# SahakyanLab/GenomeAssembler_dev

Measured on AMD Instinct MI355X. Metric: k-mers built+scored/sec, higher is better.
Workload: dtype u64 keys / u32 counts / f64 scores; 1 GPU; cfg2 (configs[2]): 100 x 50000 bp segments per GPU, 150 bp reads at 50x, k=31, build + breakage scoring of all contigs; mode=segments, segments_total=100, distinct_kmers_rank0=3843627, parallelism=segments sharded over 1 GPU(s), no collective

## Files before the change

### genomeassembler_dev_amd/csrc/capi.hip

```cpp
#include <algorithm>
#include <atomic>
#include <functional>
#include <memory>
#include <mutex>
#include <new>
#include <thread>

#include "pipeline.h"
#include "scaffolds.h"

struct gasm_strlist {
    std::vector<char> data;
    std::vector<u64> off;
};

struct gasm_contigs {
    std::vector<char> data;
    std::vector<u64> off;
    u64 rows = 0;
    std::vector<u32> perm;
    int words = 1;
    std::vector<u64> dkeys;
    std::vector<u32> dmult;
};
// ... 731 lines not shown
    HIPCHK(hipStreamSynchronize(b->ctx->stream));
    *seg_read_off = b->h_sim_seg_off.data();
    *starts = b->h_read_start.data();
    return GASM_OK;
    API_GUARD_END
}

void gasm_batch_free(gasm_batch* b) {
    if (!b) return;
    b->d_read_start.release();
    (void)hipSetDevice(b->ctx->device);
    (void)hipStreamSynchronize(b->ctx->stream);
    for (StepSlot& x : b->slot) { if (x.cx && x.cx != b->ctx) (void)hipStreamSynchronize(x.cx->stream); x.bs.release(); x.dp.release(); x.ss.release(); }
    b->rd.release(); b->rd2.release(); b->guided.release(); b->d_rkc.release(); b->d_correct.release();
    for (ScoreTable& t : b->tb) t.release();
    for (ScoreTable& t : b->mtb) t.release();
    delete b;
}

static int batch_build(gasm_batch* b, const BuildOpts& o) {
    if (!b) { gasm_set_error("batch is null"); return GASM_ERR_INVALID; }
    GCHK(build_opts_check(o));
    b->built = false; b->scored = false;
    const bool pingpong = env_int("GASM_PINGPONG", 1) != 0;
    if (pingpong && b->slot[0].cx == nullptr && b->slot[1].cx == nullptr)
        b->n_slots = std::max(2, std::min(4, env_int("GASM_STEP_SLOTS", 3)));
    if (pingpong) {
        if (b->last_k && b->last_k != o.k) for (StepSlot& x : b->slot) if (x.cx) HIPCHK(hipStreamSynchronize(x.cx->stream));
        b->cur = (b->cur + 1) % b->n_slots;
    }
    StepSlot& st = b->S();
    st.paths_ready = false; st.ss.valid = false; st.ss.launched = false;
    if (o.strands == 2 && b->rd2.strands_of != b->rd.upload_id) GCHK(b->rd2.make_both_strands(st.cx, b->rd));
    GCHK(pipeline_build(st.cx, o.strands == 2 ? b->rd2 : b->rd, st.bs, o));
    b->last_k = o.k;
    b->built = true;
    return GASM_OK;
}

int gasm_batch_build(gasm_batch* b, int k, uint64_t genome_len_hint) {
    API_GUARD_BEGIN
    BuildOpts o;
    o.k = k; o.genome_len_hint = genome_len_hint;
    return batch_build(b, o);
    API_GUARD_END
}

int gasm_batch_build_solid(gasm_batch* b, int k, uint64_t genome_len_hint, uint32_t min_count) {
    API_GUARD_BEGIN
    BuildOpts o;
    o.k = k; o.genome_len_hint = genome_len_hint; o.min_count = min_count;
    return batch_build(b, o);
    API_GUARD_END
}

int gasm_batch_build_strands(gasm_batch* b, int k, uint64_t genome_len_hint, uint32_t min_count, uint32_t strands) {
    API_GUARD_BEGIN
    BuildOpts o;
    o.k = k; o.genome_len_hint = genome_len_hint; o.min_count = min_count; o.strands = strands;
    return batch_build(b, o);
    API_GUARD_END
}

int gasm_batch_build_tips(gasm_batch* b, int k, uint64_t genome_len_hint, uint32_t min_count, uint32_t strands, uint32_t tip_len, uint32_t tip_rounds) {
    API_GUARD_BEGIN
    BuildOpts o;
// ... 616 lines not shown
```

### genomeassembler_dev_amd/csrc/kernels.h

```cpp
#pragma once
#include <hip/hip_runtime.h>
#include <stdint.h>

#include "device_utils.h"
#include "keyops.h"

struct ReadSet {
    const u64* words;
    const u64* read_off;
    const u64* seg_read_off;
    const u32* seg_tile_start;
    const uint4* tile_info;
    u32 fixed_len;
    u32 n_segments;
};

__device__ __forceinline__ void read_span(const ReadSet& rs, u64 r, u64* p0, u32* len) {
    if (rs.fixed_len) { *p0 = rs.read_off ? rs.read_off[r] : r * rs.fixed_len; *len = rs.fixed_len; }
    else { const u64 a = rs.read_off[r]; *p0 = a; *len = (u32)(rs.read_off[r + 1] - a); }
}

struct GraphView {
    const void* dk_key;
    const u32* dstart;
// ... 121 lines not shown
__global__ void k_bucket_partition(ReadSet rs, const uint4* tinfo, int k, int bbits, u32 g, u32 padm, u32 n_tiles, const u64* bstart, u32* cursor,
                                   K* keys, u64 scratch, u32* flags);
template <class K, int TBL>
__global__ void k_bucket_dedup(K* keys, u32* mult, const u64* bstart, const u32* blen, u32* bucket_d, u32* overflow, u16* fdir, int low_bits, u32* dstart);
#define GASM_BUCKET_MAX 65535
template <class K>
__global__ void k_bucket_dedup_multi(const K* keys, K* keys_out, u32* mult, const u64* bstart, u32* bucket_d, u32* overflow, u16* fdir, int low_bits);
template <class K>
__global__ void k_bucket_solid(K* keys, u32* mult, const u64* bstart, u32* bucket_d, u16* fdir, int low_bits, int fbits, int bbits, u32 min_count,
                               u32* removed, u32* done, u32* dstart);
template <class K>
__global__ void k_tip_mark(GraphView gv, u32 n_segments, u32 chunks, const u8* eflag, const u32* clen, const u32* nxt, const u32* dk_cnt, const u64* bstart,
                           u32* mult, u32 tip_len, u32* flags, u32* tips);
template <class K>
__global__ void k_bubble_mark(GraphView gv, u32 n_segments, u32 chunks, const u8* eflag, const u32* clen, const u32* nxt, const u32* dk_cnt, const u64* bstart,
                              u32* mult, u32 bubble_len, u32* flags, u32* bubbles);
__global__ void k_kmer_spectrum(const u32* dstart, u32 nb, const u32* dk_cnt, u32 n_segments, u32 chunks, u32* hist);
template <class K>
__global__ void k_lowcov_mark(GraphView gv, u32 n_segments, u32 chunks, const u8* eflag, const u32* clen, const u32* nxt, const u32* dk_cnt, const u64* bstart,
                              u32* mult, u32 cov_len, u32 cov_cutoff, u32* flags, u32* removed);
__global__ void k_contig_cov(const u32* dstart, u32 nb, u32 n_segments, u32 chunks, const u64* link, const u32* e_cid, const u32* dk_cnt,
                             const u32* seg_cstart, unsigned long long* msum, u32* nedges);
template <class K>
__global__ void k_bucket_gather(const K* keys, const u32* mult, const u64* bstart, const u32* dstart, K* dk_key, u32* dk_cnt, u32* claim, u8* eflag,
                                u32* flags);
template <class K> __global__ void k_edge_target(GraphView gv, u32 n_segments, u32 chunks, u32* tgt, u32* claim);
__global__ void k_edge_multi(GraphView gv, u32 n_segments, u32 chunks, const u32* tgt, const u32* claim, u8* eflag);
template <class K>
__global__ void k_node_flags(GraphView gv, u32 n_segments, u32 chunks, const u32* claim, u8* eflag, u64* link, u32* clen);
__global__ void k_edge_next(GraphView gv, u32 n_segments, u32 chunks, const u32* tgt, const u8* eflag, u32* nxt, u64* link);
__global__ void k_link_jump(GraphView gv, u32 n_segments, u32 chunks, u64* link, const u32* prev_active, u32* active, int jumps, const u32* nxt,
                            u32* clen);
__global__ void k_rank_rulers(GraphView gv, u32 n_segments, u32 chunks, u64* link, u32* rtab, u32 rshift, u32* flags);
__global__ void k_rank_lds(GraphView gv, const u32* rtab, u64* link, int max_rounds, u32 rshift, u32 lds_entries, u32* flags);
__global__ void k_chain_len(const u32* nxt, const u64* link, u32* clen, const u32* n_edges_p);
__global__ void k_contig_scan(GraphView gv, const u8* eflag, const u32* clen, u32* e_cid, u64* e_coff, u32* seg_ncontig,
                              u64* seg_cbases, u32* done, u32* seg_cstart, u64* seg_bstart, const u32* flags, u32* report, u32 ticket);
__global__ void k_contig_place(GraphView gv, const u8* eflag, const u32* seg_cstart, const u64* seg_bstart, u32* e_cid, u64* e_coff,
                               u64* c_off, u32 n_segments, u32 chunks);
template <class K>
__global__ void k_contig_emit(GraphView gv, const u64* link, const u32* nxt, const u64* e_coff, u8* out, u32 n_segments, u32 chunks);
__global__ void k_reads_both_strands(const u64* words, const u64* read_off, const u64* seg_read_off, u32 fixed_len, u32 n_segments, u64 n_reads, u32 g,
                                     unsigned long long* out);
template <class K>
__global__ void k_contig_twin(GraphView gv, const u64* link, const u32* e_cid, const u64* c_off, const u32* seg_cstart, const u8* text, u32 n_segments,
                              u32* twin, u32* bad);

template <class K>
__global__ void k_pack_runs(const K* keys, const u32* mult, const u64* bstart, const u32* bucket_d, const u32* gb_list, const u64* dst_off, K* out_keys,
                            u32* out_cnt);
template <class K, int TBL>
__global__ void k_bucket_merge(const K* in_keys, const u32* in_cnt, const u64* run_off, const u32* run_len, u32 n_src, K* out_keys, u32* out_cnt,
                               const u64* bstart, u32* bucket_d, u32* overflow, u16* fdir, int low_bits, const u64* src_base);
__global__ void k_repack_reads(const u64* src, const u64* dir, u64* words_out);
__global__ void k_piece_positions(const u64* piece_first, const u64* piece_word_off, u32 n_pieces, u64 n_reads, u32 fixed_len, u64* pos);
__global__ void k_slice_last(const u32* a, const u64* off, u32 n, u32* out);

__global__ void k_chain_expand(const u64* cwords, const u64* c_off, const u64* sig_off, const u32* elem_contig, const u32* elem_skip, const u64* elem_pos,
                               const u64* out_off, u32 n_scaffolds, u64* out, u64 n_words);
struct ChainSigs {
    const u64* sig_off;
    const u32* elem_contig;
    const u32* elem_skip;
    const u64* elem_pos;
};
__global__ void k_str_bitonic(const u64* words, const u64* off, u32* idx, u32 n_pow2, u32 kk, u32 j, ChainSigs cs);
__global__ void k_str_bitonic_block(const u64* words, const u64* off, u32* idx, u32 n_pow2, u32 kk, u32 j0, ChainSigs cs);
__global__ void k_str_adjacent_eq(const u64* words, const u64* off, const u32* idx, u32 n, u8* same_as_prev, ChainSigs cs);
// ... 116 lines not shown
```

### genomeassembler_dev_amd/csrc/kernels_build.hip

```cpp
#include "device_utils.h"
#include "keyops.h"
#include "kernels.h"
#include "dedup_order.h"

typedef unsigned long long u64x2 __attribute__((ext_vector_type(2)));

typedef unsigned int u32x4nt __attribute__((ext_vector_type(4)));
__device__ __forceinline__ uint4 stream_load16(const uint4* p) {
    const u32x4nt v = __builtin_nontemporal_load(reinterpret_cast<const u32x4nt*>(p));
    return make_uint4(v.x, v.y, v.z, v.w);
}
__device__ __forceinline__ void stream_store16(u64x2 v, u64x2* p) { __builtin_nontemporal_store(v, p); }

__global__ void __launch_bounds__(GASM_WG) k_pack_ascii(const u8* __restrict__ ascii, u64 nbases_host, const u64* __restrict__ nbases_dev,
                                                        u64* __restrict__ words, u32* __restrict__ err) {
    const u64 nbases = nbases_dev ? *nbases_dev : nbases_host;
    const u64 nwords = (nbases + 31) / 32 + 4;
    bool ok = true;
    for (u64 t = (u64)blockIdx.x * GASM_WG + threadIdx.x; t < nwords; t += (u64)gridDim.x * GASM_WG) {
        const u64 b0 = t << 5;
        u64 w = 0;
        if (b0 + 32 <= nbases) {
            const uint4* src = reinterpret_cast<const uint4*>(ascii + b0);
            const uint4 v0 = src[0], v1 = src[1];
// ... 1010 lines not shown
    }
}

#define GASM_RANK_NONE 0xFFFFFFFFu
__global__ void __launch_bounds__(GASM_WG) k_rank_rulers(GraphView gv, u32 n_segments, u32 chunks, u64* __restrict__ link,
                                                         u32* __restrict__ rtab, u32 rshift, u32* __restrict__ flags) {
    const u32 rmask = (1u << rshift) - 1u;
    u32 seg, chunk;
    if (!seg_chunk(n_segments, chunks, &seg, &chunk)) return;
    const u32 nb = 1u << gv.bbits;
    const u32 lo = gv.dstart[seg * nb], hi = gv.dstart[(seg + 1) * nb];
    const u32 nr = (hi - lo + rmask) >> rshift;
    for (u32 r = chunk * GASM_WG + threadIdx.x; r < nr; r += chunks * GASM_WG) {
        const u32 i = lo + (r << rshift);
        u32 cur = i, acc = 0, e = GASM_RANK_NONE;
        int step = 0;
        for (; step < 4096; ++step) {
            const u64 l = link[cur];
            if (cur != i) link[cur] = ((u64)i << 32) | GASM_LINK_TAG | acc;
            const u32 a = (u32)(l >> 32);
            if (a == GASM_NONE32) break;
            acc += (u32)l & 0x7FFFFFFFu;
            const u32 al = a - lo;
            if ((l & GASM_LINK_DONE) || !(al & rmask)) { e = (al << 16) | acc; break; }
            if (a == i) break;
            cur = a;
        }
        if (step == 4096) flags[GASM_FLAG_RANK_FAILED] = 1u;
        rtab[(lo >> rshift) + seg + r] = e;
    }
}

#define GASM_RANK_DEAD 0x8000FFFFu
__global__ void __launch_bounds__(1024) k_rank_lds(GraphView gv, const u32* __restrict__ rtab, u64* __restrict__ link, int max_rounds,
                                                    u32 rshift, u32 lds_entries, u32* __restrict__ flags) {
    const u32 rmask = (1u << rshift) - 1u;
    extern __shared__ u32 s_e[];
    __shared__ u32 s_active;
    const u32 seg = blockIdx.x;
    const u32 nb = 1u << gv.bbits;
    const u32 lo = gv.dstart[seg * nb], hi = gv.dstart[(seg + 1) * nb];
    const u32 nr = (hi - lo + rmask) >> rshift;
    if (nr > lds_entries || hi - lo > 65534u) { if (threadIdx.x == 0) flags[GASM_FLAG_RANK_FAILED] = 1u; return; }
    const u32* src = rtab + (lo >> rshift) + seg;
    u32 mine[32];
    u32 live = 0;
#pragma unroll
    for (u32 q = 0; q < 32; ++q) {
        const u32 r = threadIdx.x + 1024 * q;
        u32 e = r < nr ? src[r] : GASM_RANK_NONE;
        bool hopping = false;
        if (e == GASM_RANK_NONE) e = GASM_RANK_DEAD;
        else {
            const u32 a = e >> 16;
            if ((a & rmask) || (a == (r << rshift) && !(e & 0xFFFFu))) e = (0x8000u | r) << 16;
            else if (a == (r << rshift)) e = GASM_RANK_DEAD;
            else { e = ((a >> rshift) << 16) | (e & 0xFFFFu); hopping = true; }
        }
        mine[q] = e;
        if (r < nr) s_e[r] = e;
        live |= (u32)hopping << q;
    }
    for (int round = 0; round < max_rounds; ++round) {
        if (threadIdx.x == 0) s_active = 0;
        __syncthreads();
        u32 any = 0;
// ... 22 lines not shown
        const bool go = s_active != 0;
        __syncthreads();
        if (!go) break;
    }
#pragma unroll
    for (u32 q = 0; q < 32; ++q) {
        const u32 r = threadIdx.x + 1024 * q;
        if (r >= nr) continue;
        const u32 e = mine[q];
        u64 l = ~0ull;
        if (!((live >> q) & 1u) && e != GASM_RANK_DEAD) {
            const u32 t = (e >> 16) & 0x7FFFu;
            if (s_e[t] != GASM_RANK_DEAD) {
                const u32 ot = src[t];
                l = ((u64)(lo + (ot >> 16)) << 32) | GASM_LINK_DONE | (((e & 0xFFFFu) + (ot & 0xFFFFu)) & 0xFFFFu);
            }
        }
        link[lo + (r << rshift)] = l;
    }
}

__global__ void __launch_bounds__(GASM_WG) k_chain_len(const u32* __restrict__ nxt, const u64* __restrict__ link, u32* __restrict__ clen,
                                                       const u32* __restrict__ n_edges_p) {
    const u32 n_edges = *n_edges_p;
    for (u32 i = blockIdx.x * GASM_WG + threadIdx.x; i < n_edges; i += gridDim.x * GASM_WG) {
        if (nxt[i] != GASM_NONE32) continue;
        const u64 l = link[i];
        const u32 a = (u32)(l >> 32);
        if (a == GASM_NONE32 || !(l & GASM_LINK_DONE)) continue;
        clen[a] = ((u32)l & 0x7FFFFFFFu) + 1;
    }
}

__global__ void __launch_bounds__(1024) k_contig_scan(GraphView gv, const u8* __restrict__ eflag, const u32* __restrict__ clen,
                                                      u32* __restrict__ e_cid, u64* __restrict__ e_coff,
                                                      u32* __restrict__ seg_ncontig, u64* __restrict__ seg_cbases,
                                                      u32* __restrict__ done, u32* __restrict__ seg_cstart, u64* __restrict__ seg_bstart,
                                                      const u32* __restrict__ flags, u32* __restrict__ report, u32 ticket) {
    __shared__ u32 s_last;
    __shared__ u32 s_cnt[16];
    __shared__ u64 s_bas[16];
    const u32 seg = blockIdx.x;
    const u32 nb = 1u << gv.bbits;
    const u32 lo = gv.dstart[seg * nb], hi = gv.dstart[(seg + 1) * nb];
    const u32 wv = threadIdx.x >> 6, ln = threadIdx.x & 63;
    const u32 per = ((hi - lo + 15) / 16 + 63) & ~63u;
    const u32 wa = min(hi, lo + wv * per), wb = min(hi, wa + per);
    u32 ccarry = 0;
    u64 bcarry = 0;
    for (u32 base = wa; base < wb; base += 1024) {
        u32 ef[16];
        u32 cl[16];
#pragma unroll
        for (u32 q = 0; q < 16; ++q) {
            const u32 i = base + q * 64 + ln;
            ef[q] = i < wb ? (u32)eflag[i] : 0u;
            cl[q] = i < wb ? clen[i] : 0u;
        }
#pragma unroll
        for (u32 q = 0; q < 16; ++q) __asm__ volatile("" : "+v"(cl[q]), "+v"(ef[q]));
#pragma unroll
        for (u32 q = 0; q < 16; ++q) {
            const u32 i = base + q * 64 + ln;
            const bool head = ef[q] & 1;
            const u32 len = head ? (u32)(gv.k - 1) + cl[q] : 0u;
            const u32 cinc = wave_incl_scan(head ? 1u : 0u);
            const u32 binc = wave_incl_scan(len);
            if (head) { e_cid[i] = ccarry + cinc - 1; e_coff[i] = bcarry + binc - len; }
            ccarry += wave_last(cinc);
            bcarry += wave_last(binc);
        }
    }
    if (ln == 0) { s_cnt[wv] = ccarry; s_bas[wv] = bcarry; }
    __syncthreads();
    u32 cbefore = 0, ctot = 0;
    u64 bbefore = 0, btot = 0;
#pragma unroll
    for (u32 w = 0; w < 16; ++w) {
        if (w < wv) { cbefore += s_cnt[w]; bbefore += s_bas[w]; }
        ctot += s_cnt[w]; btot += s_bas[w];
    }
    if (wv) {
        for (u32 base = wa + ln; base < wb; base += 2048) {
            u32 ef[32];
#pragma unroll
            for (u32 q = 0; q < 32; ++q) ef[q] = base + 64 * q < wb ? (u32)eflag[base + 64 * q] : 0u;
#pragma unroll
            for (u32 q = 0; q < 32; ++q)
                if (ef[q] & 1) { e_cid[base + 64 * q] += cbefore; e_coff[base + 64 * q] += bbefore; }
        }
    }
    if (threadIdx.x == 0) {
        publish_u32(&seg_ncontig[seg], ctot); publish_u64(&seg_cbases[seg], btot);
        s_last = count_in_last(done) ? 1u : 0u;
    }
    __syncthreads();
    if (!s_last || wv) return;
    seg_offsets_wave(seg_ncontig, seg_cbases, gridDim.x, seg_cstart, seg_bstart, gv.dstart, nb, flags, report, ticket);
}

__global__ void __launch_bounds__(GASM_WG) k_contig_place(GraphView gv, const u8* __restrict__ eflag,
                                                          const u32* __restrict__ seg_cstart, const u64* __restrict__ seg_bstart,
                                                          u32* __restrict__ e_cid, u64* __restrict__ e_coff,
                                                          u64* __restrict__ c_off, u32 n_segments, u32 chunks) {
    if (blockIdx.x == 0 && threadIdx.x == 0) c_off[seg_cstart[n_segments]] = seg_bstart[n_segments];
    for_seg_edges(gv.dstart, 1u << gv.bbits, n_segments, chunks, [&](u32 seg, u32, u32, u32 i) {
        if (!(eflag[i] & 1)) return;
        const u32 cid = seg_cstart[seg] + e_cid[i];
        const u64 off = seg_bstart[seg] + e_coff[i];
        e_cid[i] = cid;
        e_coff[i] = off;
        c_off[cid] = off;
    });
}

__device__ __forceinline__ u32 klow16(u64 a) { return (u32)a & 0xFFFFu; }
__device__ __forceinline__ u32 klow16(const K128& a) { return (u32)a.lo & 0xFFFFu; }
template <class K>
__global__ void __launch_bounds__(GASM_WG) k_contig_emit(GraphView gv, const u64* __restrict__ link, const u32* __restrict__ nxt,
                                                         const u64* __restrict__ e_coff, u8* __restrict__ out, u32 n_segments,
                                                         u32 chunks) {
    for_seg_edge_groups(gv.dstart, 1u << gv.bbits, n_segments, chunks, [&](u32, u32, u32, const u32 (&i)[GASM_EDGE_ILP], const bool (&ok)[GASM_EDGE_ILP]) {
        u64 l[GASM_EDGE_ILP], off[GASM_EDGE_ILP];
        u32 nx[GASM_EDGE_ILP];
        K key[GASM_EDGE_ILP];
        bool on[GASM_EDGE_ILP];
        const int k = gv.k;
        const bool wide = k >= 8;
#pragma unroll
        for (int q = 0; q < GASM_EDGE_ILP; ++q) {
            l[q] = ok[q] ? link[i[q]] : ~0ull;
            nx[q] = ok[q] ? nxt[i[q]] : 0u;
// ... 288 lines not shown
```

### genomeassembler_dev_amd/csrc/pipeline.h

```cpp
#pragma once
#include "gasm_internal.h"
#include "kernels.h"

template <class K> struct KeyTag { using type = K; };
template <class F> static inline int with_key(int words, F&& f) { return words == 1 ? f(KeyTag<u64>{}) : f(KeyTag<K128>{}); }
#define GLAUNCH_K(ctx, words, name, kern, grid, block, shmem, ...)          \
    GCHK(with_key(words, [&](auto _tag) -> int {                            \
        using K = typename decltype(_tag)::type;                            \
        GLAUNCH(ctx, name, kern, grid, block, shmem, __VA_ARGS__);          \
        return GASM_OK;                                                     \
    }))

struct DevReads {
    u32 n_segments = 0;
    u64 n_reads = 0, total_bases = 0;
    u32 fixed_len = 0;
    u32 min_len = 0, max_len = 0;
    u64 n_empty = 0;
    std::vector<u64> h_read_off;
    std::vector<u64> h_seg_read_off;
    std::vector<u64> h_seg_empty;
    bool positioned = false;
    int sim_shift = 52;
    u64 upload_id = 0;
// ... 75 lines not shown
    }
    template <class T> T* at(const DBuf& d, size_t i) const { return reinterpret_cast<T*>(static_cast<char*>(d.p) + t[i].off); }
};
struct PassState {
    DBuf d;
    std::vector<std::vector<u64>> h;
    bool queued = false;
    u32 param[2] = {0, 0};
    template <class T> const T* host(size_t i) const { return reinterpret_cast<const T*>(h[i].data()); }
};
enum { LINKS_SUCC, LINKS_PRED, LINKS_LSUP, LINKS_SSUP, LINKS_SKIPPED };
enum { PAIRS_REC, PAIRS_HIST, PAIRS_CNT };
enum { MAP_REC, MAP_PILE, MAP_HIST, MAP_CNT };
enum { MAPG_REC, MAPG_GAP, MAPG_PILE, MAPG_GPILE, MAPG_HIST, MAPG_CNT, MAPG_END, MAPG_ENDCNT };
enum { MAPSC_F64, MAPSC_I32, MAPSC_CNT, MAPSC_FX, MAPSC_PILE, MAPSC_COUNTERS };

struct BuildState {
    int k = 0, bbits = 0, fbits = 9, words = 1, bb_cap = 0;
    bool small_tbl = true;
    bool rank_global = false;
    bool single_pass = true;
    struct PartLayout {
        u64 reads_id = 0;
        int k = 0, bbits = 0, slack = 0, forced = 0;
        u32 padm = 0, g = 0;
        bool operator==(const PartLayout& o) const {
            return reads_id == o.reads_id && k == o.k && bbits == o.bbits && slack == o.slack && forced == o.forced && padm == o.padm && g == o.g;
        }
    } part;
    bool part_valid = false;
    u64 part_alloc = 0;
    bool multi_pass = false;
    bool ranked_in_lds = false;
    u32 tile_g = 1;
    u64 n_kmers = 0, hint = 0, reads_id = 0;
    BuildOpts opts;
    std::vector<u64> h_seg_nk;
    u64 D_cap = 0, maxD_cap = 0, bases_cap = 0;
    u32 maxD_est = 1, paths_est = 0;
    bool have_actual = false;
    u32 tile_orr = 1;
    bool part_single = false;
    bool scan_in_dedup = false;
    u32 ruler_shift = 0;
    u32 attempts_distinct = 0;
    u32 attempts_graph = 0;
    u32* h_report = nullptr;
    size_t h_report_words = 0;
    u32 ticket = 0;
    bool pending = false;
    u32 d_total = 0, n_contigs = 0;
    u64 contig_bases = 0;
    std::vector<u32> h_dstart;
    std::vector<u32> h_seg_cstart;
    std::vector<u64> h_seg_bstart;
    DBuf d_keys2;
    DBuf d_keys, d_mult, d_hist, d_toff, d_tcnt, d_fdir, d_bstart, d_bucket_d, d_dstart, d_flags, d_rtab;
    DBuf d_solid_removed;
    RoundStats round_stats[ROUND_KINDS] = {{GASM_MAX_TIP_ROUNDS}, {GASM_MAX_BUBBLE_ROUNDS}, {GASM_MAX_COV_ROUNDS}};
    DBuf d_ccov;
    std::vector<u64> h_ccov_m;
    std::vector<u32> h_ccov_n;
    bool coverage_queued = false;
    PassState links, pairs, map, mapg;
    PassState mapscore;
    int mapscore_shift[GASM_MAX_TABLES] = {};
// ... 100 lines not shown
```

### genomeassembler_dev_amd/csrc/pipeline.hip

```cpp
#include <atomic>
#include <chrono>
#include <thread>
#include "pipeline.h"

#include <algorithm>
#include <cmath>

__global__ void k_set_u64(u64* p, u64 v) { *p = v; }

__global__ void k_add_empty_reads(PathSet ps, const u64* __restrict__ seg_empty, u32* __restrict__ poscnt, u32* __restrict__ total) {
    const u32 seg = blockIdx.y;
    const u32 p = ps.seg_path_off[seg] + blockIdx.x * GASM_WG + threadIdx.x;
    if (p >= ps.seg_path_off[seg + 1]) return;
    const u32 e = (u32)seg_empty[seg];
    if (!e) return;
    if (ps.p_off[p + 1] > ps.p_off[p]) poscnt[ps.p_off[p]] += e;
    else total[p] += e;
}

struct Knobs {
    int dedup_tbl = 0, scatter_wgs = 8, hist_wgs = 64, rank_rounds = 18, bbits_add = 0, ruler_shift = 0;
    bool rank_global = false, sync_build = false;
    Knobs() {
        if (const char* v = getenv("GASM_DEDUP_TBL")) dedup_tbl = atoi(v);
        if (const char* v = getenv("GASM_SCATTER_WGS")) scatter_wgs = std::max(1, atoi(v));
        if (const char* v = getenv("GASM_HIST_WGS")) hist_wgs = std::max(1, atoi(v));
        if (const char* v = getenv("GASM_DBG_BBITS_ADD")) bbits_add = std::max(0, atoi(v));
        if (const char* v = getenv("GASM_RULER_SHIFT")) ruler_shift = std::min(4, std::max(0, atoi(v)));
        if (const char* v = getenv("GASM_DBG_RANK_ROUNDS")) rank_rounds = atoi(v);
        rank_global = getenv("GASM_RANK_GLOBAL") != nullptr;
        sync_build = getenv("GASM_SYNC_BUILD") != nullptr;
    }
};
static const Knobs& knobs() { static const Knobs k; return k; }

template <class T>
static int wait_word(gasm_ctx* ctx, const volatile T* word, T ticket) {
    const auto t0 = std::chrono::steady_clock::now();
    for (u32 spin = 0;; ++spin) {
        if (*word == ticket) { std::atomic_thread_fence(std::memory_order_acquire); return GASM_OK; }
        if ((spin & 1023u) == 1023u && std::chrono::steady_clock::now() - t0 > std::chrono::milliseconds(2)) break;
    }
    static const double limit_s = [] { const char* v = getenv("GASM_WAIT_TIMEOUT_S"); const double x = v && *v ? atof(v) : 300.0; return x > 0 ? x : 300.0; }();
    for (;;) {
        if (*word == ticket) { std::atomic_thread_fence(std::memory_order_acquire); return GASM_OK; }
        const hipError_t q = hipStreamQuery(ctx->stream);
        if (q == hipSuccess) break;
        if (q != hipErrorNotReady) { gasm_set_error("the stream failed while a report was awaited: %s", hipGetErrorString(q)); return GASM_ERR_HIP; }
        if (std::chrono::duration<double>(std::chrono::steady_clock::now() - t0).count() > limit_s) {
            gasm_set_error("no report from the device within %.0f s (GASM_WAIT_TIMEOUT_S): a kernel hangs or the GPU is lost", limit_s);
            return GASM_ERR_HIP;
        }
        std::this_thread::sleep_for(std::chrono::microseconds(50));
    }
    if (*word != ticket) { gasm_set_error("a kernel finished without writing its report"); return GASM_ERR_HIP; }
    std::atomic_thread_fence(std::memory_order_acquire);
    return GASM_OK;
}
int gasm_wait_word32(gasm_ctx* ctx, const volatile u32* word, u32 ticket) { return wait_word<u32>(ctx, word, ticket); }
int gasm_wait_word64(gasm_ctx* ctx, const volatile u64* word, u64 ticket) { return wait_word<u64>(ctx, word, ticket); }
static int wait_report(gasm_ctx* ctx, const volatile u32* word, u32 ticket) { return wait_word<u32>(ctx, word, ticket); }
// ... 338 lines not shown
    v.p_off = b_p_off ? b_p_off : d_p_off.as<u64>();
    v.seg_path_off = b_seg_path_off ? b_seg_path_off : d_seg_path_off.as<u32>();
    v.n_segments = n_segments;
    return v;
}

void DevPaths::release() { d_words.release(); d_p_off.release(); d_seg_path_off.release(); d_seg_base_off.release(); }

void BuildState::release() {
    for (DBuf* b : {&d_solid_removed, &d_ccov, &links.d, &pairs.d, &map.d, &mapg.d, &mapscore.d, &d_spectrum, &d_twin, &d_keys, &d_keys2, &d_mult, &d_hist, &d_toff, &d_tcnt, &d_fdir, &d_bstart, &d_bucket_d, &d_dstart, &d_flags, &d_dk_key, &d_dk_cnt,
                    &d_eflag, &d_nxt, &d_link, &d_clen, &d_ecid, &d_ecoff, &d_rtab, &d_seg_cbases, &d_seg_cstart,
                    &d_seg_bstart, &d_c_off, &d_contig_ascii})
        b->release();
    for (RoundStats& rs : round_stats) rs.d_stats.release();
    part_valid = false;
    if (h_report) { (void)hipHostFree(h_report); h_report = nullptr; h_report_words = 0; }
}

void ScoreState::release() {
    for (DBuf* b : {&d_tbl_off, &d_seed, &d_gpos, &d_poscnt, &d_total, &d_out_f64, &d_out_i32, &d_freq, &d_pd_off, &d_pd, &d_seg_empty, &d_fxsum, &d_first, &d_first_off}) b->release();
}

static int ensure_lds_attrs(gasm_ctx* ctx) {
    if (ctx->lds_attrs_set) return GASM_OK;
#define GASM_LDS_ATTR(kern, bytes) HIPCHK(hipFuncSetAttribute(reinterpret_cast<const void*>(kern), hipFuncAttributeMaxDynamicSharedMemorySize, bytes));
#define GASM_SCORE_LDS_ATTR(T) GASM_LDS_ATTR((k_score_reads_graph<K, T>), GASM_SCORE_PATH_CAP * 12)
    for (int words = 1; words <= 2; ++words)
        GCHK(with_key(words, [&](auto tag) -> int {
            using K = typename decltype(tag)::type;
            GASM_LDS_ATTR(k_bucket_scatter<K>, 160 * 1024) GASM_LDS_ATTR(k_bucket_partition<K>, 160 * 1024) GASM_LDS_ATTR(k_tile_hist<K>, 160 * 1024)
            GASM_SCORE_LDS_ATTR(1) GASM_SCORE_LDS_ATTR(2) GASM_SCORE_LDS_ATTR(3) GASM_SCORE_LDS_ATTR(4) GASM_SCORE_LDS_ATTR(5) GASM_SCORE_LDS_ATTR(6) GASM_SCORE_LDS_ATTR(7) GASM_SCORE_LDS_ATTR(8)
            return GASM_OK;
        }));
    GASM_LDS_ATTR(k_rank_lds, 160 * 1024 - 64)
#define GASM_MAPSCORE_LDS_ATTR(T) GASM_LDS_ATTR((k_score_mapped<T, false>), GASM_SCORE_PATH_CAP * 12) GASM_LDS_ATTR((k_score_mapped<T, true>), GASM_SCORE_PATH_CAP * 12)
    GASM_MAPSCORE_LDS_ATTR(1) GASM_MAPSCORE_LDS_ATTR(2) GASM_MAPSCORE_LDS_ATTR(3) GASM_MAPSCORE_LDS_ATTR(4) GASM_MAPSCORE_LDS_ATTR(5) GASM_MAPSCORE_LDS_ATTR(6)
    GASM_MAPSCORE_LDS_ATTR(7) GASM_MAPSCORE_LDS_ATTR(8)
#undef GASM_MAPSCORE_LDS_ATTR
#undef GASM_SCORE_LDS_ATTR
#undef GASM_LDS_ATTR
    ctx->lds_attrs_set = true;
    return GASM_OK;
}

void distinct_caps(BuildState& bs, u32 S) {
    const u64 limit = bs.multi_pass ? GASM_BUCKET_MAX : bs.small_tbl ? GASM_TBL_LIMIT / 2 : GASM_TBL_LIMIT;
    const u64 per_seg = ((u64)1 << bs.bbits) * limit;
    const u64 all = bs.k < 16 ? ((u64)1 << (2 * bs.k)) : ~(u64)0;
    bs.D_cap = 0; bs.maxD_cap = 0;
    for (u32 s = 0; s < S; ++s) {
        const u64 c = std::min(std::min(bs.h_seg_nk[s], per_seg), all);
        bs.D_cap += c;
        bs.maxD_cap = std::max(bs.maxD_cap, c);
    }
}

static int launch_graph_dense(gasm_ctx* ctx, u32 S, BuildState& bs, bool last_pass);

static GraphView graph_view(const BuildState& bs) {
    GraphView gv;
    gv.dk_key = bs.d_dk_key.p;
    gv.dstart = bs.d_dstart.as<u32>();
    gv.fdir = bs.d_fdir.as<u16>();
    gv.k = bs.k;
    gv.bbits = bs.bbits;
    gv.fbits = bs.fbits;
    return gv;
// ... 165 lines not shown
            GLAUNCH_K(ctx, W, "k_tip_mark", k_tip_mark<K>, seg_grid(dchunks, S), dim3(GASM_WG), 0, graph_view(bs), S, dchunks, bs.d_eflag.as<u8>(), bs.d_clen.as<u32>(),
                      bs.d_nxt.as<u32>(), bs.d_dk_cnt.as<u32>(), bs.d_bstart.as<u64>(), bs.d_mult.as<u32>(), o.tip_len, bs.d_flags.as<u32>(), d_contigs);
        } else if (kind == ROUNDS_BUBBLE) {
            GLAUNCH_K(ctx, W, "k_bubble_mark", k_bubble_mark<K>, seg_grid(dchunks, S), dim3(GASM_WG), 0, graph_view(bs), S, dchunks, bs.d_eflag.as<u8>(),
                      bs.d_clen.as<u32>(), bs.d_nxt.as<u32>(), bs.d_dk_cnt.as<u32>(), bs.d_bstart.as<u64>(), bs.d_mult.as<u32>(), o.bubble_len,
                      bs.d_flags.as<u32>(), d_contigs);
        } else {
            GLAUNCH_K(ctx, W, "k_lowcov_mark", k_lowcov_mark<K>, seg_grid(dchunks, S), dim3(GASM_WG), 0, graph_view(bs), S, dchunks, bs.d_eflag.as<u8>(),
                      bs.d_clen.as<u32>(), bs.d_nxt.as<u32>(), bs.d_dk_cnt.as<u32>(), bs.d_bstart.as<u64>(), bs.d_mult.as<u32>(), o.cov_len, o.cov_cutoff,
                      bs.d_flags.as<u32>(), d_contigs);
        }
        u32* const d_scan_out = bs.scan_in_dedup ? bs.d_dstart.as<u32>() : nullptr;
        GLAUNCH_K(ctx, W, "k_bucket_solid", k_bucket_solid<K>, dim3(nbt), dim3(GASM_WG), 0, bs.d_keys.as<K>(), bs.d_mult.as<u32>(), bs.d_bstart.as<u64>(),
                  bs.d_bucket_d.as<u32>(), bs.d_fdir.as<u16>(), 2 * bs.k - bbits, bs.fbits, bbits, 1u, d_kmers, bs.d_flags.as<u32>() + GASM_FLAG_SOLID_DONE, d_scan_out);
        if (!d_scan_out) GLAUNCH(ctx, "k_scan_excl", k_scan_excl<u32>, dim3(1), dim3(1024), 0, bs.d_bucket_d.as<u32>(), bs.d_dstart.as<u32>(), nbt);
    }
    return GASM_OK;
}

static int launch_graph_dense(gasm_ctx* ctx, u32 S, BuildState& bs, bool last_pass) {
    GasmRange range("gasm:graph (degrees, list ranking, contigs)");
    const int W = bs.words;
    u32* const d_claim = bs.d_nxt.as<u32>();
    u32* const d_seg_ncontig = reinterpret_cast<u32*>(bs.d_seg_cbases.as<u64>() + S);
    u32* const d_fl = bs.d_flags.as<u32>();
    const GraphView gv = graph_view(bs);
    const u32 nb = 1u << bs.bbits;
    const u32 est = std::max<u32>(1, (u32)std::min<u64>(bs.maxD_est, bs.maxD_cap));
    const u32 dchunks = (u32)ceil_div_u64(est, GASM_WG);
    const dim3 grid_seg = seg_grid(dchunks, S);
    const u32 gchunks = (u32)ceil_div_u64(est, GASM_WG * GASM_EDGE_ILP);
    const dim3 grid_grp = seg_grid(gchunks, S);
    u32* const d_tgt = bs.d_ecid.as<u32>();
    GLAUNCH_K(ctx, W, "k_edge_target", k_edge_target<K>, grid_seg, dim3(GASM_WG), 0, gv, S, dchunks, d_tgt, d_claim);
    GLAUNCH(ctx, "k_edge_multi", k_edge_multi, grid_grp, dim3(GASM_WG), 0, gv, S, gchunks, d_tgt, d_claim, bs.d_eflag.as<u8>());
    GLAUNCH_K(ctx, W, "k_node_flags", k_node_flags<K>, grid_seg, dim3(GASM_WG), 0, gv, S, dchunks, d_claim, bs.d_eflag.as<u8>(), bs.d_link.as<u64>(), bs.d_clen.as<u32>());
    GLAUNCH(ctx, "k_edge_next", k_edge_next, grid_grp, dim3(GASM_WG), 0, gv, S, gchunks, d_tgt, bs.d_eflag.as<u8>(), bs.d_nxt.as<u32>(), bs.d_link.as<u64>());
    u32* const act = d_fl + GASM_FLAG_ACTIVE;
    const u32 jchunks = (u32)ceil_div_u64(est, GASM_WG * GASM_JUMP_ILP);
    bs.ranked_in_lds = est <= 65534 && !bs.rank_global && !knobs().rank_global;
    bs.ruler_shift = 0;
    if (bs.ranked_in_lds) {
        const u32 rshift = knobs().ruler_shift ? (u32)knobs().ruler_shift : (S >= (u32)ctx->n_cu / 4 ? 1u : 2u);
        bs.ruler_shift = rshift;
        const u32 rchunks = (u32)ceil_div_u64((est + (1u << rshift) - 1) >> rshift, GASM_WG);
        u32 lds_entries = 32767;
        if (S > (u32)ctx->n_cu) lds_entries = std::min<u32>(32767, (((est + est / 4) >> rshift) + 1024) & ~1023u);
        GLAUNCH(ctx, "k_rank_rulers", k_rank_rulers, seg_grid(rchunks, S), dim3(GASM_WG), 0, gv, S, rchunks, bs.d_link.as<u64>(), bs.d_rtab.as<u32>(), rshift, d_fl);
        GLAUNCH(ctx, "k_rank_lds", k_rank_lds, dim3(S), dim3(1024), (size_t)lds_entries * 4 + 4, gv, bs.d_rtab.as<u32>(), bs.d_link.as<u64>(), knobs().rank_rounds, rshift,
                lds_entries, d_fl);
        const int jumps = 255, launches = 2;
        static_assert(launches <= GASM_FLAG_ACTIVE_N, "an active word per launch");
        for (int r = 0; r < launches; ++r)
            GLAUNCH(ctx, "k_link_jump", k_link_jump, seg_grid(jchunks, S), dim3(GASM_WG), 0, gv, S, jchunks, bs.d_link.as<u64>(), r ? act + r - 1 : nullptr, act + r, jumps,
                    bs.d_nxt.as<u32>(), bs.d_clen.as<u32>());
    } else {
        int rounds = 1;
        while ((1ull << rounds) < bs.maxD_cap) ++rounds;
        rounds += 1;
        const int jumps = 4, launches = (rounds * 10 + 22) / 23 + 1;
        if (launches > (int)GASM_FLAG_ACTIVE_N) { gasm_set_error("segment too large for the list-ranking flags"); return GASM_ERR_CAPACITY; }
        for (int r = 0; r < launches; ++r)
            GLAUNCH(ctx, "k_link_jump", k_link_jump, seg_grid(jchunks, S), dim3(GASM_WG), 0, gv, S, jchunks, bs.d_link.as<u64>(), r ? act + r - 1 : nullptr, act + r, jumps,
                    (const u32*)nullptr, (u32*)nullptr);
    }
    const u32 grid_all = (u32)std::min<u64>(ceil_div_u64((u64)est * S, GASM_WG), (u64)ctx->n_cu * 64);
    if (!bs.ranked_in_lds)
        GLAUNCH(ctx, "k_chain_len", k_chain_len, dim3(std::max(1u, grid_all)), dim3(GASM_WG), 0, bs.d_nxt.as<u32>(), bs.d_link.as<u64>(),
                bs.d_clen.as<u32>(), gv.dstart + (size_t)S * nb);
    if (!last_pass) return GASM_OK;
    const size_t words = BuildReport<u32>::words(S);
    if (bs.h_report_words < words) {
        if (bs.h_report) (void)hipHostFree(bs.h_report);
        bs.h_report = nullptr; bs.h_report_words = 0;
        HIPCHK(hipHostMalloc((void**)&bs.h_report, words * 4, hipHostMallocCoherent));
        bs.h_report_words = words;
    }
    bs.ticket = next_ticket();
    BuildReport<volatile u32>{bs.h_report, S}.ticket() = 0;
    GLAUNCH(ctx, "k_contig_scan", k_contig_scan, dim3(S), dim3(1024), 0, gv, bs.d_eflag.as<u8>(), bs.d_clen.as<u32>(),
            bs.d_ecid.as<u32>(), bs.d_ecoff.as<u64>(), d_seg_ncontig, bs.d_seg_cbases.as<u64>(), d_fl + GASM_FLAG_CONTIG_DONE, bs.d_seg_cstart.as<u32>(),
            bs.d_seg_bstart.as<u64>(), d_fl, bs.h_report, bs.ticket);
    GLAUNCH(ctx, "k_contig_place", k_contig_place, grid_seg, dim3(GASM_WG), 0, gv, bs.d_eflag.as<u8>(),
            bs.d_seg_cstart.as<u32>(), bs.d_seg_bstart.as<u64>(), bs.d_ecid.as<u32>(), bs.d_ecoff.as<u64>(), bs.d_c_off.as<u64>(), S, dchunks);
    GLAUNCH_K(ctx, W, "k_contig_emit", k_contig_emit<K>, grid_grp, dim3(GASM_WG), 0, gv, bs.d_link.as<u64>(), bs.d_nxt.as<u32>(),
              bs.d_ecoff.as<u64>(), bs.d_contig_ascii.as<u8>(), S, gchunks);
    bs.pending = true;
    return GASM_OK;
}

int plan_build(gasm_ctx* ctx, DevReads& rd, int k, u64 hint, BuildState& bs) {
    if (k < 2 || k > GASM_MAX_K) { gasm_set_error("k = %d not supported (2..%d)", k, GASM_MAX_K); return GASM_ERR_INVALID; }
    const int W = k <= 31 ? 1 : 2;
    const u32 KT = (u32)with_key(W, [](auto tag) -> int { return KeyTraits<typename decltype(tag)::type>::KT; });
    HIPCHK(hipSetDevice(ctx->device));
    GCHK(ensure_lds_attrs(ctx));
    const u32 S = rd.n_segments;
    const bool same = bs.k == k && bs.words == W && bs.h_seg_nk.size() == S && bs.hint == hint && bs.reads_id == rd.upload_id;
    bs.words = W; bs.k = k; bs.hint = hint; bs.reads_id = rd.upload_id;
    bs.fetched_distinct = bs.fetched_contigs = false;
    bs.pending = false;
    u64 N = 0, maxNs = 0;
    bs.h_seg_nk.assign(S, 0);
    if (rd.fixed_len) {
        const u64 nk = rd.fixed_len >= (u32)k ? rd.fixed_len - k + 1 : 0;
        for (u32 s = 0; s < S; ++s) bs.h_seg_nk[s] = (rd.h_seg_read_off[s + 1] - rd.h_seg_read_off[s]) * nk;
    } else {
        u32 s = 0;
        for (u64 r = 0; r < rd.n_reads; ++r) {
            while (r >= rd.h_seg_read_off[s + 1]) ++s;
            const u64 L = rd.h_read_off[r + 1] - rd.h_read_off[r];
            if (L >= (u64)k) bs.h_seg_nk[s] += L - k + 1;
        }
    }
    for (u64 v : bs.h_seg_nk) { N += v; maxNs = std::max(maxNs, v); }
// ... 1101 lines not shown
```

Measured before the change: 234.6 billion k-mers/s.

## Use narrow 512-thread workgroups for LDS ranking and contig scan when pipelined

Adds a 512-thread variant of the LDS list-ranking kernel that keeps per-thread liveness bitmasks and processes entries in batches of eight, plus a templated contig scan that can run with 8 waves. When the batch runs on ping-pong step slots and there are enough segments, these narrow variants are chosen and the LDS allocation is sized to the segment instead of the maximum. The aim is to let several segments' tail kernels share a CU and overlap with other slots' work, rather than one 1024-thread, LDS-heavy block per CU. The cost is more serial work per thread and more registers per thread, and a new, more complex ranking path that could be wrong at edge cases.

Result: no change. 235.7 billion k-mers/s (median of 3 runs) (+0.5%).

```diff
diff --git a/genomeassembler_dev_amd/csrc/capi.hip b/genomeassembler_dev_amd/csrc/capi.hip
--- a/genomeassembler_dev_amd/csrc/capi.hip
+++ b/genomeassembler_dev_amd/csrc/capi.hip
@@ -787,6 +787,7 @@
     StepSlot& st = b->S();
     st.paths_ready = false; st.ss.valid = false; st.ss.launched = false;
     if (o.strands == 2 && b->rd2.strands_of != b->rd.upload_id) GCHK(b->rd2.make_both_strands(st.cx, b->rd));
+    st.bs.on_slots = pingpong;
     GCHK(pipeline_build(st.cx, o.strands == 2 ? b->rd2 : b->rd, st.bs, o));
     b->last_k = o.k;
     b->built = true;
diff --git a/genomeassembler_dev_amd/csrc/kernels.h b/genomeassembler_dev_amd/csrc/kernels.h
--- a/genomeassembler_dev_amd/csrc/kernels.h
+++ b/genomeassembler_dev_amd/csrc/kernels.h
@@ -177,8 +177,11 @@
 __global__ void k_link_jump(GraphView gv, u32 n_segments, u32 chunks, u64* link, const u32* prev_active, u32* active, int jumps, const u32* nxt,
                             u32* clen);
 __global__ void k_rank_rulers(GraphView gv, u32 n_segments, u32 chunks, u64* link, u32* rtab, u32 rshift, u32* flags);
+constexpr int GASM_TAIL_NARROW_WG = 512;
 __global__ void k_rank_lds(GraphView gv, const u32* rtab, u64* link, int max_rounds, u32 rshift, u32 lds_entries, u32* flags);
+__global__ void k_rank_lds_narrow(GraphView gv, const u32* rtab, u64* link, int max_rounds, u32 rshift, u32 lds_entries, u32* flags);
 __global__ void k_chain_len(const u32* nxt, const u64* link, u32* clen, const u32* n_edges_p);
+template <int WAVES>
 __global__ void k_contig_scan(GraphView gv, const u8* eflag, const u32* clen, u32* e_cid, u64* e_coff, u32* seg_ncontig,
                               u64* seg_cbases, u32* done, u32* seg_cstart, u64* seg_bstart, const u32* flags, u32* report, u32 ticket);
 __global__ void k_contig_place(GraphView gv, const u8* eflag, const u32* seg_cstart, const u64* seg_bstart, u32* e_cid, u64* e_coff,
diff --git a/genomeassembler_dev_amd/csrc/kernels_build.hip b/genomeassembler_dev_amd/csrc/kernels_build.hip
--- a/genomeassembler_dev_amd/csrc/kernels_build.hip
+++ b/genomeassembler_dev_amd/csrc/kernels_build.hip
@@ -1066,6 +1066,106 @@
 }
 
 #define GASM_RANK_DEAD 0x8000FFFFu
+__global__ void __launch_bounds__(GASM_TAIL_NARROW_WG, 4)
+k_rank_lds_narrow(GraphView gv, const u32* __restrict__ rtab, u64* __restrict__ link, int max_rounds, u32 rshift, u32 lds_entries, u32* __restrict__ flags) {
+    constexpr u32 NT = GASM_TAIL_NARROW_WG;
+    constexpr u32 C = 32768 / (NT * 32);
+    const u32 rmask = (1u << rshift) - 1u;
+    extern __shared__ u32 s_e[];
+    __shared__ u32 s_active;
+    const u32 seg = blockIdx.x;
+    const u32 nb = 1u << gv.bbits;
+    const u32 lo = gv.dstart[seg * nb], hi = gv.dstart[(seg + 1) * nb];
+    const u32 nr = (hi - lo + rmask) >> rshift;
+    if (nr > lds_entries || hi - lo > 65534u) { if (threadIdx.x == 0) flags[GASM_FLAG_RANK_FAILED] = 1u; return; }
+    const u32* src = rtab + (lo >> rshift) + seg;
+    u32 live[C];
+#pragma unroll
+    for (u32 c = 0; c < C; ++c) {
+        live[c] = 0;
+#pragma unroll 1
+        for (u32 q0 = 0; q0 < 32 && NT * (32 * c + q0) < nr; q0 += 8) {
+            u32 e8[8];
+#pragma unroll
+            for (u32 u = 0; u < 8; ++u) { const u32 r = threadIdx.x + NT * (32 * c + q0 + u); e8[u] = r < nr ? src[r] : GASM_RANK_NONE; }
+#pragma unroll
+            for (u32 u = 0; u < 8; ++u) {
+                const u32 r = threadIdx.x + NT * (32 * c + q0 + u);
+                u32 e = e8[u];
+                bool hopping = false;
+                if (e == GASM_RANK_NONE) e = GASM_RANK_DEAD;
+                else {
+                    const u32 a = e >> 16;
+                    if ((a & rmask) || (a == (r << rshift) && !(e & 0xFFFFu))) e = (0x8000u | r) << 16;
+                    else if (a == (r << rshift)) e = GASM_RANK_DEAD;
+                    else { e = ((a >> rshift) << 16) | (e & 0xFFFFu); hopping = true; }
+                }
+                if (r < nr) s_e[r] = e;
+                live[c] |= (u32)hopping << (q0 + u);
+            }
+        }
+    }
+    for (int round = 0; round < max_rounds; ++round) {
+        if (threadIdx.x == 0) s_active = 0;
+        __syncthreads();
+        u32 any = 0;
+#pragma unroll
+        for (u32 c = 0; c < C; ++c) {
+#pragma unroll 1
+            for (u32 q0 = 0; q0 < 32; q0 += 8) {
+                if (((live[c] >> q0) & 0xFFu) == 0) continue;
+                u32 e8[8], x[8];
+#pragma unroll
+                for (u32 u = 0; u < 8; ++u) {
+                    const u32 r = threadIdx.x + NT * (32 * c + q0 + u);
+                    e8[u] = r < nr ? s_e[r] : GASM_RANK_DEAD;
+                }
+#pragma unroll
+                for (u32 u = 0; u < 8; ++u) x[u] = s_e[(e8[u] >> 16) & 0x7FFFu];
+#pragma unroll
+                for (u32 u = 0; u < 8; ++u) {
+                    const u32 q = q0 + u;
+                    const u32 r = threadIdx.x + NT * (32 * c + q), e = e8[u];
+                    const u32 lv = (live[c] >> q) & 1u, stop = x[u] >> 31;
+                    const u32 hop = lv & ~stop;
+                    const u32 hopped = (x[u] & 0xFFFF0000u) | ((e + x[u]) & 0xFFFFu);
+                    const u32 ne = hop ? hopped : e;
+                    live[c] &= ~((lv & stop) << q);
+                    any |= hop;
+                    s_e[min(r, nr)] = ne;
+                }
+            }
+        }
+        if (any) s_active = 1;
+        __syncthreads();
+        const bool go = s_active != 0;
+        __syncthreads();
+        if (!go) break;
+    }
+#pragma unroll
+    for (u32 c = 0; c < C; ++c) {
+#pragma unroll 1
+        for (u32 q0 = 0; q0 < 32 && NT * (32 * c + q0) < nr; q0 += 8) {
+#pragma unroll
+            for (u32 u = 0; u < 8; ++u) {
+                const u32 q = q0 + u;
+                const u32 r = threadIdx.x + NT * (32 * c + q);
+                if (r >= nr) continue;
+                const u32 e = s_e[r];
+                u64 l = ~0ull;
+                if (!((live[c] >> q) & 1u) && e != GASM_RANK_DEAD) {
+                    const u32 t = (e >> 16) & 0x7FFFu;
+                    if (s_e[t] != GASM_RANK_DEAD) {
+                        const u32 ot = src[t];
+                        l = ((u64)(lo + (ot >> 16)) << 32) | GASM_LINK_DONE | (((e & 0xFFFFu) + (ot & 0xFFFFu)) & 0xFFFFu);
+                    }
+                }
+                link[lo + (r << rshift)] = l;
+            }
+        }
+    }
+}
+
 __global__ void __launch_bounds__(1024) k_rank_lds(GraphView gv, const u32* __restrict__ rtab, u64* __restrict__ link, int max_rounds,
                                                     u32 rshift, u32 lds_entries, u32* __restrict__ flags) {
     const u32 rmask = (1u << rshift) - 1u;
@@ -1154,35 +1254,38 @@
     }
 }
 
-__global__ void __launch_bounds__(1024) k_contig_scan(GraphView gv, const u8* __restrict__ eflag, const u32* __restrict__ clen,
-                                                      u32* __restrict__ e_cid, u64* __restrict__ e_coff,
-                                                      u32* __restrict__ seg_ncontig, u64* __restrict__ seg_cbases,
-                                                      u32* __restrict__ done, u32* __restrict__ seg_cstart, u64* __restrict__ seg_bstart,
-                                                      const u32* __restrict__ flags, u32* __restrict__ report, u32 ticket) {
+template <int WAVES>
+__global__ void __launch_bounds__(WAVES * 64, WAVES == 16 ? 4 : 8)
+k_contig_scan(GraphView gv, const u8* __restrict__ eflag, const u32* __restrict__ clen, u32* __restrict__ e_cid, u64* __restrict__ e_coff,
+              u32* __restrict__ seg_ncontig, u64* __restrict__ seg_cbases, u32* __restrict__ done, u32* __restrict__ seg_cstart, u64* __restrict__ seg_bstart,
+              const u32* __restrict__ flags, u32* __restrict__ report, u32 ticket) {
+    static_assert(WAVES == 16 || WAVES == 8, "waves per workgroup");
+    constexpr u32 ROWS = WAVES == 16 ? 16 : 8;
+    constexpr u32 ROWS2 = WAVES == 16 ? 32 : 12;
     __shared__ u32 s_last;
-    __shared__ u32 s_cnt[16];
-    __shared__ u64 s_bas[16];
+    __shared__ u32 s_cnt[WAVES];
+    __shared__ u64 s_bas[WAVES];
     const u32 seg = blockIdx.x;
     const u32 nb = 1u << gv.bbits;
     const u32 lo = gv.dstart[seg * nb], hi = gv.dstart[(seg + 1) * nb];
     const u32 wv = threadIdx.x >> 6, ln = threadIdx.x & 63;
-    const u32 per = ((hi - lo + 15) / 16 + 63) & ~63u;
+    const u32 per = ((hi - lo + WAVES - 1) / WAVES + 63) & ~63u;
     const u32 wa = min(hi, lo + wv * per), wb = min(hi, wa + per);
     u32 ccarry = 0;
     u64 bcarry = 0;
-    for (u32 base = wa; base < wb; base += 1024) {
-        u32 ef[16];
-        u32 cl[16];
-#pragma unroll
-        for (u32 q = 0; q < 16; ++q) {
+    for (u32 base = wa; base < wb; base += 64 * ROWS) {
+        u32 ef[ROWS];
+        u32 cl[ROWS];
+#pragma unroll
+        for (u32 q = 0; q < ROWS; ++q) {
             const u32 i = base + q * 64 + ln;
             ef[q] = i < wb ? (u32)eflag[i] : 0u;
             cl[q] = i < wb ? clen[i] : 0u;
         }
 #pragma unroll
-        for (u32 q = 0; q < 16; ++q) __asm__ volatile("" : "+v"(cl[q]), "+v"(ef[q]));
-#pragma unroll
-        for (u32 q = 0; q < 16; ++q) {
+        for (u32 q = 0; q < ROWS; ++q) __asm__ volatile("" : "+v"(cl[q]), "+v"(ef[q]));
+#pragma unroll
+        for (u32 q = 0; q < ROWS; ++q) {
             const u32 i = base + q * 64 + ln;
             const bool head = ef[q] & 1;
             const u32 len = head ? (u32)(gv.k - 1) + cl[q] : 0u;
@@ -1198,17 +1301,17 @@
     u32 cbefore = 0, ctot = 0;
     u64 bbefore = 0, btot = 0;
 #pragma unroll
-    for (u32 w = 0; w < 16; ++w) {
+    for (u32 w = 0; w < WAVES; ++w) {
         if (w < wv) { cbefore += s_cnt[w]; bbefore += s_bas[w]; }
         ctot += s_cnt[w]; btot += s_bas[w];
     }
     if (wv) {
-        for (u32 base = wa + ln; base < wb; base += 2048) {
-            u32 ef[32];
-#pragma unroll
-            for (u32 q = 0; q < 32; ++q) ef[q] = base + 64 * q < wb ? (u32)eflag[base + 64 * q] : 0u;
-#pragma unroll
-            for (u32 q = 0; q < 32; ++q)
+        for (u32 base = wa + ln; base < wb; base += 64 * ROWS2) {
+            u32 ef[ROWS2];
+#pragma unroll
+            for (u32 q = 0; q < ROWS2; ++q) ef[q] = base + 64 * q < wb ? (u32)eflag[base + 64 * q] : 0u;
+#pragma unroll
+            for (u32 q = 0; q < ROWS2; ++q)
                 if (ef[q] & 1) { e_cid[base + 64 * q] += cbefore; e_coff[base + 64 * q] += bbefore; }
         }
     }
@@ -1220,6 +1323,9 @@
     if (!s_last || wv) return;
     seg_offsets_wave(seg_ncontig, seg_cbases, gridDim.x, seg_cstart, seg_bstart, gv.dstart, nb, flags, report, ticket);
 }
+#define GASM_CONTIG_SCAN_INST(W) template __global__ void k_contig_scan<W>(GraphView, const u8*, const u32*, u32*, u64*, u32*, u64*, u32*, u32*, u64*, const u32*, u32*, u32);
+GASM_CONTIG_SCAN_INST(16) GASM_CONTIG_SCAN_INST(GASM_TAIL_NARROW_WG / 64)
+#undef GASM_CONTIG_SCAN_INST
 
 __global__ void __launch_bounds__(GASM_WG) k_contig_place(GraphView gv, const u8* __restrict__ eflag,
                                                           const u32* __restrict__ seg_cstart, const u64* __restrict__ seg_bstart,
diff --git a/genomeassembler_dev_amd/csrc/pipeline.h b/genomeassembler_dev_amd/csrc/pipeline.h
--- a/genomeassembler_dev_amd/csrc/pipeline.h
+++ b/genomeassembler_dev_amd/csrc/pipeline.h
@@ -131,6 +131,7 @@
     u64 part_alloc = 0;
     bool multi_pass = false;
     bool ranked_in_lds = false;
+    bool on_slots = false;
     u32 tile_g = 1;
     u64 n_kmers = 0, hint = 0, reads_id = 0;
     BuildOpts opts;
diff --git a/genomeassembler_dev_amd/csrc/pipeline.hip b/genomeassembler_dev_amd/csrc/pipeline.hip
--- a/genomeassembler_dev_amd/csrc/pipeline.hip
+++ b/genomeassembler_dev_amd/csrc/pipeline.hip
@@ -19,14 +19,13 @@
 }
 
 struct Knobs {
-    int dedup_tbl = 0, scatter_wgs = 8, hist_wgs = 64, rank_rounds = 18, bbits_add = 0, ruler_shift = 0;
+    int dedup_tbl = 0, scatter_wgs = 8, hist_wgs = 64, rank_rounds = 18, bbits_add = 0;
     bool rank_global = false, sync_build = false;
     Knobs() {
         if (const char* v = getenv("GASM_DEDUP_TBL")) dedup_tbl = atoi(v);
         if (const char* v = getenv("GASM_SCATTER_WGS")) scatter_wgs = std::max(1, atoi(v));
         if (const char* v = getenv("GASM_HIST_WGS")) hist_wgs = std::max(1, atoi(v));
         if (const char* v = getenv("GASM_DBG_BBITS_ADD")) bbits_add = std::max(0, atoi(v));
-        if (const char* v = getenv("GASM_RULER_SHIFT")) ruler_shift = std::min(4, std::max(0, atoi(v)));
         if (const char* v = getenv("GASM_DBG_RANK_ROUNDS")) rank_rounds = atoi(v);
         rank_global = getenv("GASM_RANK_GLOBAL") != nullptr;
         sync_build = getenv("GASM_SYNC_BUILD") != nullptr;
@@ -431,7 +430,7 @@
             GASM_SCORE_LDS_ATTR(1) GASM_SCORE_LDS_ATTR(2) GASM_SCORE_LDS_ATTR(3) GASM_SCORE_LDS_ATTR(4) GASM_SCORE_LDS_ATTR(5) GASM_SCORE_LDS_ATTR(6) GASM_SCORE_LDS_ATTR(7) GASM_SCORE_LDS_ATTR(8)
             return GASM_OK;
         }));
-    GASM_LDS_ATTR(k_rank_lds, 160 * 1024 - 64)
+    GASM_LDS_ATTR(k_rank_lds, 160 * 1024 - 64) GASM_LDS_ATTR(k_rank_lds_narrow, 160 * 1024 - 64)
 #define GASM_MAPSCORE_LDS_ATTR(T) GASM_LDS_ATTR((k_score_mapped<T, false>), GASM_SCORE_PATH_CAP * 12) GASM_LDS_ATTR((k_score_mapped<T, true>), GASM_SCORE_PATH_CAP * 12)
     GASM_MAPSCORE_LDS_ATTR(1) GASM_MAPSCORE_LDS_ATTR(2) GASM_MAPSCORE_LDS_ATTR(3) GASM_MAPSCORE_LDS_ATTR(4) GASM_MAPSCORE_LDS_ATTR(5) GASM_MAPSCORE_LDS_ATTR(6)
     GASM_MAPSCORE_LDS_ATTR(7) GASM_MAPSCORE_LDS_ATTR(8)
@@ -663,6 +662,8 @@
     const u32 gchunks = (u32)ceil_div_u64(est, GASM_WG * GASM_EDGE_ILP);
     const dim3 grid_grp = seg_grid(gchunks, S);
     u32* const d_tgt = bs.d_ecid.as<u32>();
+    bool tail_narrow = bs.on_slots && S >= (u32)ctx->n_cu / 4;
+    if (const int forced = env_int("GASM_TAIL_WG", 0)) tail_narrow = forced == GASM_TAIL_NARROW_WG;
     GLAUNCH_K(ctx, W, "k_edge_target", k_edge_target<K>, grid_seg, dim3(GASM_WG), 0, gv, S, dchunks, d_tgt, d_claim);
     GLAUNCH(ctx, "k_edge_multi", k_edge_multi, grid_grp, dim3(GASM_WG), 0, gv, S, gchunks, d_tgt, d_claim, bs.d_eflag.as<u8>());
     GLAUNCH_K(ctx, W, "k_node_flags", k_node_flags<K>, grid_seg, dim3(GASM_WG), 0, gv, S, dchunks, d_claim, bs.d_eflag.as<u8>(), bs.d_link.as<u64>(), bs.d_clen.as<u32>());
@@ -672,14 +673,18 @@
     bs.ranked_in_lds = est <= 65534 && !bs.rank_global && !knobs().rank_global;
     bs.ruler_shift = 0;
     if (bs.ranked_in_lds) {
-        const u32 rshift = knobs().ruler_shift ? (u32)knobs().ruler_shift : (S >= (u32)ctx->n_cu / 4 ? 1u : 2u);
+        const u32 forced_shift = (u32)std::min(4, std::max(0, env_int("GASM_RULER_SHIFT", 0)));
+        const u32 rshift = forced_shift ? forced_shift : (S >= (u32)ctx->n_cu / 4 ? 1u : 2u);
         bs.ruler_shift = rshift;
         const u32 rchunks = (u32)ceil_div_u64((est + (1u << rshift) - 1) >> rshift, GASM_WG);
         u32 lds_entries = 32767;
-        if (S > (u32)ctx->n_cu) lds_entries = std::min<u32>(32767, (((est + est / 4) >> rshift) + 1024) & ~1023u);
+        if (tail_narrow || S > (u32)ctx->n_cu) lds_entries = std::min<u32>(32767, (((est + est / 4) >> rshift) + 1024) & ~1023u);
+        const size_t lds_bytes = (size_t)lds_entries * 4 + 4;
         GLAUNCH(ctx, "k_rank_rulers", k_rank_rulers, seg_grid(rchunks, S), dim3(GASM_WG), 0, gv, S, rchunks, bs.d_link.as<u64>(), bs.d_rtab.as<u32>(), rshift, d_fl);
-        GLAUNCH(ctx, "k_rank_lds", k_rank_lds, dim3(S), dim3(1024), (size_t)lds_entries * 4 + 4, gv, bs.d_rtab.as<u32>(), bs.d_link.as<u64>(), knobs().rank_rounds, rshift,
-                lds_entries, d_fl);
+        if (tail_narrow)
+            GLAUNCH(ctx, "k_rank_lds", k_rank_lds_narrow, dim3(S), dim3(GASM_TAIL_NARROW_WG), lds_bytes, gv, bs.d_rtab.as<u32>(), bs.d_link.as<u64>(), knobs().rank_rounds, rshift, lds_entries, d_fl);
+        else
+            GLAUNCH(ctx, "k_rank_lds", k_rank_lds, dim3(S), dim3(1024), lds_bytes, gv, bs.d_rtab.as<u32>(), bs.d_link.as<u64>(), knobs().rank_rounds, rshift, lds_entries, d_fl);
         const int jumps = 255, launches = 2;
         static_assert(launches <= GASM_FLAG_ACTIVE_N, "an active word per launch");
         for (int r = 0; r < launches; ++r)
@@ -709,9 +714,14 @@
     }
     bs.ticket = next_ticket();
     BuildReport<volatile u32>{bs.h_report, S}.ticket() = 0;
-    GLAUNCH(ctx, "k_contig_scan", k_contig_scan, dim3(S), dim3(1024), 0, gv, bs.d_eflag.as<u8>(), bs.d_clen.as<u32>(),
-            bs.d_ecid.as<u32>(), bs.d_ecoff.as<u64>(), d_seg_ncontig, bs.d_seg_cbases.as<u64>(), d_fl + GASM_FLAG_CONTIG_DONE, bs.d_seg_cstart.as<u32>(),
-            bs.d_seg_bstart.as<u64>(), d_fl, bs.h_report, bs.ticket);
+    if (tail_narrow)
+        GLAUNCH(ctx, "k_contig_scan", k_contig_scan<GASM_TAIL_NARROW_WG / 64>, dim3(S), dim3(GASM_TAIL_NARROW_WG), 0, gv, bs.d_eflag.as<u8>(), bs.d_clen.as<u32>(),
+                bs.d_ecid.as<u32>(), bs.d_ecoff.as<u64>(), d_seg_ncontig, bs.d_seg_cbases.as<u64>(), d_fl + GASM_FLAG_CONTIG_DONE, bs.d_seg_cstart.as<u32>(),
+                bs.d_seg_bstart.as<u64>(), d_fl, bs.h_report, bs.ticket);
+    else
+        GLAUNCH(ctx, "k_contig_scan", k_contig_scan<16>, dim3(S), dim3(1024), 0, gv, bs.d_eflag.as<u8>(), bs.d_clen.as<u32>(),
+                bs.d_ecid.as<u32>(), bs.d_ecoff.as<u64>(), d_seg_ncontig, bs.d_seg_cbases.as<u64>(), d_fl + GASM_FLAG_CONTIG_DONE, bs.d_seg_cstart.as<u32>(),
+                bs.d_seg_bstart.as<u64>(), d_fl, bs.h_report, bs.ticket);
     GLAUNCH(ctx, "k_contig_place", k_contig_place, grid_seg, dim3(GASM_WG), 0, gv, bs.d_eflag.as<u8>(),
             bs.d_seg_cstart.as<u32>(), bs.d_seg_bstart.as<u64>(), bs.d_ecid.as<u32>(), bs.d_ecoff.as<u64>(), bs.d_c_off.as<u64>(), S, dchunks);
     GLAUNCH_K(ctx, W, "k_contig_emit", k_contig_emit<K>, grid_grp, dim3(GASM_WG), 0, gv, bs.d_link.as<u64>(), bs.d_nxt.as<u32>(),
```
